# dmlc/xgboost

Hardware: AMD Instinct MI355X
Metric: boosting_rounds_per_sec (higher is better)
Workload: dtype fp32; 1 GPU; model=higgs-1m-hist, rows_per_gpu=1000000, n_features=28, max_depth=8, max_bin=256, objective=binary:logistic, parallelism=dp1, device=cuda

## Files before the change

### xgboost_amd/backend/gpu.py

```python
from __future__ import annotations

from typing import List, Optional, Sequence, Tuple

import numpy as np
import torch

from .. import collective
from ..data import QuantizedMatrix
from ..params import TrainParam
from ..splits import SplitEntry, feature_set_mask
from .cpu import GradQuantizer

LDS_MAX_GROUP_BINS = 8192
TARGET_HIST_TASKS = 2048
MIN_ROWS_PER_TASK = 1024
HIST_MAX_GROUP_FEATURES = 1024


def _check_bin_dtype(gidx: torch.Tensor) -> None:
    if gidx.dtype not in (torch.uint8, torch.int16):
        raise ValueError(
            f"GPU kernels take uint8 or 16-bit bin matrices, got "
            f"{gidx.dtype}: a feature has more than 65535 local bin ids "
            f"(lower max_bin or the category count, or train on the CPU)")
# ... 455 lines not shown
        c8, c16, cld = self._gidx_col_args()
        self.lib.gbt_partition(
            p8, p16, self.qm.n_features, c8, c16, cld, self.hip.ptr(ridx),
            self.hip.ptr(self._ridx_out), self.hip.ptr(tasks), len(tasks_np),
            self.hip.ptr(feat_t), self.hip.ptr(sbin_t), self.hip.ptr(dleft_t),
            self.hip.ptr(cat_bits_t), self.hip.ptr(cat_off_t),
            self.hip.ptr(self.n_bins_feat), self.hip.ptr(cnt_t),
            self.hip.stream())
        self.lib.gbt_copy_ranges(
            self.hip.ptr(self._ridx_out), self.hip.ptr(ridx),
            self.hip.ptr(tasks), len(tasks_np), self.hip.stream())
        final = cnt_t.cpu().numpy()
        out = []
        for i, (s, e) in enumerate(segments):
            mid = int(final[i, 0])
            assert mid == int(final[i, 1]), (
                f"partition counters disagree: {final[i]}")
            out.append(((s, mid), (mid, e)))
        return out

    def grow_tree_native(self, qgpair: torch.Tensor, tree, param,
                         quantizer, monotone: Optional[np.ndarray],
                         root_sums: torch.Tensor,
                         feature_mask: Optional[np.ndarray] = None):
        import ctypes
        if not hasattr(self.lib, "gbt_grow_tree"):
            return None
        if param.max_depth <= 0 or param.max_depth > 14:
            return None
        n_rows = qgpair.shape[0]
        max_build = max(1, 1 << max(param.max_depth - 2, 0))
        pool_rows = 2 * max_build
        pool_bytes = pool_rows * self.n_bins * 16
        if pool_bytes > (32 << 30):
            return None
        dev = self.device
        ws = getattr(self, "_native_ws", None)
        if ws is None or ws["pool_rows"] < pool_rows or ws["n"] < n_rows:
            ws = {
                "pool_rows": pool_rows, "n": n_rows,
                "ridx": torch.empty(n_rows, dtype=torch.int32, device=dev),
                "ridx_out": torch.empty(n_rows, dtype=torch.int32,
                                        device=dev),
                "pool_a": torch.empty((pool_rows, self.n_bins, 2),
                                      dtype=torch.int64, device=dev),
                "pool_b": torch.empty((pool_rows, self.n_bins, 2),
                                      dtype=torch.int64, device=dev),
# ... 63 lines not shown
                       for t in (ws["pool_a"], ws["pool_b"])]
            if ws["wt_ws"] is not None:
                w = ws["wt_ws"]
                regions.append((w.data_ptr(), w.numel(), w))

            def _allreduce(ptr, n_elems):
                addr = ctypes.addressof(ptr.contents)
                for base, nbytes, t in regions:
                    if base <= addr < base + nbytes:
                        off = addr - base
                        i64 = t.view(torch.uint8).view(-1)[
                            off:off + 8 * n_elems].view(torch.int64)
                        collective.allreduce_sum_(i64)
                        return
                raise RuntimeError("allreduce pointer outside workspaces")

            cb = self.hip.ALLREDUCE_FN(_allreduce)
        p8, p16 = self._gidx_ptrs()
        c8, c16, cld = self._gidx_col_args()
        ma = getattr(quantizer, "maxabs_dev", None)
        out_scales = np.zeros(2, dtype=np.float64)
        gsc = quantizer.g_scale if ma is None else 0.0
        hsc = quantizer.h_scale if ma is None else 0.0
        qg_st = ws["qg_stage"][:n_rows]
        qg_st.copy_(qgpair.view(n_rows, 2))
        ws["rs_stage"].copy_(root_sums.view(-1)[:2])
        if ma is not None:
            ws["ma_stage"].copy_(ma.view(-1)[:2])
        rc = self.lib.gbt_grow_tree(
            ws["driver"], p8, p16, self.qm.n_features, c8, c16, n_rows,
            self.hip.ptr(qg_st),
            self.hip.ptr(self.cut_ptrs),
            cut_values_host.ctypes.data_as(ctypes.c_void_p),
            cut_ptrs_host.ctypes.data_as(ctypes.c_void_p),
            self.hip.ptr(self.n_bins_feat),
            self.hip.ptr(self.feat_group_start),
            self.hip.ptr(self.bin_group_start), self.n_groups,
            self.max_group_bins, self.use_shared, self.n_bins,
            self.hip.ptr(ws["ridx"]), self.hip.ptr(ws["ridx_out"]),
            self.hip.ptr(ws["pool_a"]), self.hip.ptr(ws["pool_b"]),
            self.hip.ptr(ws["eval_gain"]), self.hip.ptr(ws["eval_bin"]),
            self.hip.ptr(ws["eval_dir"]), self.hip.ptr(ws["eval_lsum"]),
            self.hip.ptr(ws["eval_best"]), self.hip.ptr(ws["pos"]),
            max_build,
            self.hip.ptr(ws["hist_tasks"]), ws["hist_tasks_cap"],
            self.hip.ptr(ws["wt_ws"]),
            0 if ws["wt_ws"] is None else ws["wt_ws"].numel(),
            ws["wt_max_ptasks"],
            self.hip.ptr(ws["rs_stage"]),
            self.hip.ptr(ws["ma_stage"]) if ma is not None else None,
            out_scales.ctypes.data_as(ctypes.c_void_p),
            gsc, hsc,
            param.reg_lambda, param.reg_alpha, param.max_delta_step,
            param.min_child_weight, param.gamma, param.eta, param.max_depth,
            mono_dev, mono_host, fmask_ptr, cb,
            *[host[k].ctypes.data_as(ctypes.c_void_p) for k in (
                "left", "right", "parent", "split_index", "split_cond",
                "default_left", "loss_chg", "sum_hess", "base_weight")],
            self.hip.stream())
        if rc in (-9998, -9999):
            return None
        if rc <= 0:
            raise RuntimeError(f"gbt_grow_tree failed: rc={rc}")
        if ma is not None:
            quantizer.g_scale = float(out_scales[0])
            quantizer.h_scale = float(out_scales[1])
        n = rc
        tree._ensure(n)
        tree.n_nodes = n
        tree.left[:n] = host["left"][:n]
        tree.right[:n] = host["right"][:n]
        tree.parent[:n] = host["parent"][:n]
        tree.split_index[:n] = host["split_index"][:n]
# ... 722 lines not shown
```

### xgboost_amd/core.py

```python
from __future__ import annotations

import json
import os
from typing import Any, Dict, List, Optional, Sequence, Tuple

import numpy as np
import torch

from . import collective
from .backend.cpu import CpuOps, GradQuantizer
from .data import DMatrix
from .grower import TreeGrower
from .metrics import create_metric
from .objectives import Objective, create_objective
from .params import (TrainParam, canonicalize, check_unknown,
                     make_train_param)
from .tree_model import RegTree

VERSION = (3, 5, 0)


def _resolve_device(params: Dict[str, Any]) -> torch.device:
    dev = str(params.get("device", "cpu"))
    if "device" not in params and params.get("gpu_id") is not None:
# ... 463 lines not shown
        lib.gbt_gpair_fused(
            obj_id, hip_ops.ptr(margin.contiguous().view(-1)),
            hip_ops.ptr(ent["labels"]), hip_ops.ptr(ent["weights"]),
            spw, n, hip_ops.ptr(ent["gh"]), hip_ops.ptr(ent["maxabs"]),
            hip_ops.stream())
        m = ent["maxabs"]
        if collective.is_distributed():
            collective.allreduce_max_(m)
        quantizer = GradQuantizer.__new__(GradQuantizer)
        quantizer.g_scale = None
        quantizer.h_scale = None
        quantizer.maxabs_dev = m
        if "rootsum" not in ent:
            ent["rootsum"] = torch.zeros(2, dtype=torch.int64,
                                         device=margin.device)
        else:
            ent["rootsum"].zero_()
        lib.gbt_quantize(hip_ops.ptr(ent["gh"]), n, 0.0, 0.0,
                         hip_ops.ptr(m), hip_ops.ptr(ent["qg"]),
                         hip_ops.ptr(ent["rootsum"]), hip_ops.stream())
        if collective.is_distributed():
            collective.allreduce_sum_(ent["rootsum"])
        quantizer.root_sums_dev = ent["rootsum"]
        seed = (self.seed + iteration if not self.seed_per_iteration
                else self.seed + iteration * 2654435761)
        tree = RegTree(self.n_features)
        grower = TreeGrower(ops, self.tparam, quantizer, n, seed=seed,
                            monotone=self._monotone_array(),
                            interaction=tp.interaction_constraints,
                            feature_weights=dtrain.info.feature_weights)
        tree, positions = grower.grow(ent["qg"], tree)
        self.trees.append(tree)
        self.tree_info.append(0)
        self.iteration_indptr.append(self.iteration_indptr[-1] + 1)
        leaf_np = tree.split_cond[:tree.n_nodes].copy()
        if hasattr(ops, "stager") and hasattr(lib, "gbt_margin_add") \
                and positions.device == margin.device:
            (leaf_vals,) = ops.stager.upload([leaf_np])
            mc = margin.contiguous()
            lib.gbt_margin_add(hip_ops.ptr(mc), hip_ops.ptr(positions),
                               hip_ops.ptr(leaf_vals), n,
                               mc.stride(0), 0, hip_ops.stream())
            if mc.data_ptr() != margin.data_ptr():
                margin.copy_(mc)
        else:
            leaf_vals = torch.as_tensor(leaf_np, device=margin.device)
# ... 928 lines not shown
```

### xgboost_amd/grower.py

```python
from __future__ import annotations

import dataclasses
import heapq
from typing import Dict, List, Optional, Sequence, Tuple

import numpy as np
import torch

from .backend.cpu import GradQuantizer
from .params import TrainParam
from .splits import SplitEntry, calc_weight, feature_set_mask
from .tree_model import RegTree


class ColumnSampler:

    def __init__(self, n_features: int, param: TrainParam, seed: int,
                 feature_weights: Optional[np.ndarray] = None):
        self.rng = np.random.RandomState(seed & 0x7FFFFFFF)
        self.n_features = n_features
        self.param = param
        self.weights = (np.asarray(feature_weights, dtype=np.float64)
                        if feature_weights is not None else None)
        feats = np.arange(n_features)
# ... 115 lines not shown
        p = self.param
        ops = self.ops
        if not hasattr(ops, "grow_tree_native"):
            return None
        if (self.cat_mask is not None or self.interaction is not None
                or p.colsample_bylevel < 1.0 or p.colsample_bynode < 1.0):
            return None
        fmask = None
        if p.colsample_bytree < 1.0:
            fmask = np.zeros(ops.qm.n_features, np.uint8)
            fmask[self.col_sampler.tree_set] = 1
        needs_replay = p.grow_policy == "lossguide" or p.max_leaves > 0
        if needs_replay:
            if p.max_depth <= 0 or p.max_depth > 14:
                return None
            if p.max_leaves > 0 and (1 << p.max_depth) > 16 * p.max_leaves:
                return None
        rs = getattr(self.quantizer, "root_sums_dev", None)
        if rs is None:
            from . import collective
            rs = qgpair.to(torch.int64).sum(dim=0).contiguous()
            if collective.is_distributed():
                collective.allreduce_sum_(rs)
        out = ops.grow_tree_native(qgpair, tree, p, self.quantizer,
                                   self.monotone, rs, feature_mask=fmask)
        if out is None or not needs_replay:
            return out
        dtree, pos = out
        return self._policy_replay(dtree, pos, p)

    def _policy_replay(self, dt: RegTree, pos: torch.Tensor,
                       param) -> Tuple[RegTree, torch.Tensor]:
        import heapq
        n = dt.n_nodes
        internal = dt.left[:n] >= 0
        gains = getattr(dt, "_gain64", None)
        if gains is None:
            gains = dt.loss_chg[:n].astype(np.float64)
        nt = RegTree(dt.n_features)
        nt._ensure(n)
        new_of = np.full(n, -1, np.int32)
        new_of[0] = 0
        nt.base_weight[0] = dt.base_weight[0]
        nt.sum_hess[0] = dt.sum_hess[0]
        nt.left[0] = nt.right[0] = nt.parent[0] = -1
        state = {"n_new": 1, "n_leaves": 1, "seq": 0}
        heap: List[Tuple[float, int, int, int]] = []

# ... 485 lines not shown
```

### xgboost_amd/ops/__init__.py

```python
from __future__ import annotations

import ctypes
import os
from typing import Optional

import torch

_HERE = os.path.dirname(os.path.abspath(__file__))
_LIB_PATH = os.path.join(_HERE, "libgbt_hip.so")
_lib: Optional[ctypes.CDLL] = None

_c = ctypes
_p = _c.c_void_p
_i = _c.c_int
_i64 = _c.c_int64
_f = _c.c_float
_d = _c.c_double

_SIGS = {
    "gbt_hist": [_p, _p, _i, _p, _p, _p, _i, _p, _i, _p, _p, _i, _i, _p, _i, _p, _p],
    "gbt_partition": [_p, _p, _i, _p, _p, _i64, _p, _p, _p, _i, _p, _p, _p,
                      _p, _p, _p, _p, _p],
    "gbt_evaluate_masked": [_p, _i, _i, _i, _p, _p, _p, _d, _d, _d, _d, _d,
                            _d, _p, _p, _i, _p, _p, _p, _p, _p, _p, _p, _i,
                            _p],
    "gbt_evaluate_ref": [_p, _i, _i, _i, _p, _p, _p, _d, _d, _d, _d, _d,
                         _d, _p, _p, _i, _p, _p, _p, _p, _p, _p, _p, _i,
                         _p],
    "gbt_compress": [_p, _i64, _i, _p, _p, _p, _f, _i, _p, _p, _p],
    "gbt_predict": [_p, _i64, _i, _f, _i, _p, _p, _p, _p, _p, _p, _p, _p,
                    _p, _p, _i, _i, _p, _p, _p],
    "gbt_predict_q": [_p, _i, _i64, _i, _f, _i, _p, _p, _p, _p, _p, _p, _p,
                      _p, _i, _i, _p, _p, _p],
    "gbt_predict_csr": [_p, _p, _p, _i64, _i, _p, _p, _p, _p, _p, _p, _p,
                        _i, _i, _p, _p, _i, _i, _p],
    "gbt_leaf_partition": [_p, _p, _i, _p, _p, _p],
    "gbt_leaf_decide": [_p, _p, _i, _p, _p, _i64, _p, _p, _i, _p, _p, _p,
                        _p, _p, _p, _p],
    "gbt_copy_ranges": [_p, _p, _p, _i, _p],
    "gbt_select_best": [_p, _p, _p, _p, _i, _i, _p, _p, _p],
    "gbt_mt_evaluate": [_p, _i, _i, _i, _i, _p, _p, _p, _p,
                        _d, _d, _d, _d, _p, _p, _p, _p, _p],
    "gbt_gpair_fused": [_i, _p, _p, _p, _f, _i64, _p, _p, _p],
    "gbt_quantize": [_p, _i64, _d, _d, _p, _p, _p, _p],
    "gbt_margin_add": [_p, _p, _p, _i64, _i, _i, _p],
    "gbt_hist_cpu": [_p, _p, _i, _p, _p, _p, _p, _i, _p, _p, _i],
    "gbt_partition_cpu": [_p, _p, _i, _p, _i64, _i64, _i, _i, _i, _p, _i,
                          _i, _p],
    "gbt_evaluate_cpu": [_p, _i, _i, _i, _p, _p, _d, _d, _d, _d, _d, _d,
                         _p, _p, _p, _p],
# ... 97 lines not shown
```

### xgboost_amd/ops/cpp/driver.hip

```cpp
#include "gbt_kernels.h"

#include <hip/hip_runtime.h>

#include <algorithm>
#include <cmath>
#include <cstdio>
#include <cstdlib>
#include <cstring>
#include <vector>

namespace {

#define HIP_CHECK(x)                                    \
  do {                                                  \
    hipError_t err__ = (x);                             \
    if (err__ != hipSuccess) return -(int)err__;        \
  } while (0)

constexpr int kErrReplayDiverged = -9991;
constexpr int kErrRootTasksCap = -9996;
constexpr int kErrArenaTooSmall = -9997;
constexpr int kCapacityTaskGenLds = -9998;
constexpr int kCapacityHistPool = -9999;

// ... 132 lines not shown
    readback_cap = want;
    return 0;
  }
  ~DriverCtx() {
    for (int i = 0; i < PinnedRing::kSlots; ++i) {
      if (ring.host[i]) hipHostFree(ring.host[i]);
      if (ring.dev[i]) hipFree(ring.dev[i]);
    }
    if (readback_host) hipHostFree(readback_host);
    if (wt_graph) (void)hipGraphExecDestroy(wt_graph);
    if (gstream) (void)hipStreamDestroy(gstream);
    if (gevent) (void)hipEventDestroy(gevent);
  }
};

bool WtGraphEnabled() {
  static int v = [] {
    const char* e = getenv("GBT_WT_GRAPH");
    return e ? atoi(e) : 1;
  }();
  return v != 0;
}

constexpr long long kHistMinRows = 2048;
long long HistTasksTarget() {
  static long long v = [] {
    const char* e = getenv("GBT_HIST_TASKS");
    long long t = e ? atoll(e) : 256;
    return t >= 64 && t <= 16384 ? t : 256;
  }();
  return v;
}

long long PartMinRows() {
  static long long v = [] {
    const char* e = getenv("GBT_PART_ROWS");
    long long r = e ? atoll(e) : 4096;
    return r >= 1024 && r <= 65536 && (r & (r - 1)) == 0 ? r : 4096;
  }();
  return v;
}

struct Node {
  int nid;
  int seg_begin, seg_end;
  long long gq, hq;
// ... 173 lines not shown
  }
  __syncthreads();
  const long long rpt = s_rpt;
  const int total_tasks = s_total_tasks;
  for (int t = threadIdx.x; t < max_tasks; t += blockDim.x) {
    if (t >= total_tasks) {
      out_tasks[t] = BlockTask{0, 0, 0, 0};
      continue;
    }
    int lo = 0, hi = k - 1;
    while (lo < hi) {
      const int mid = (lo + hi + 1) >> 1;
      if (s_pref[mid] <= t) lo = mid; else hi = mid - 1;
    }
    const int j = lo;
    const long long idx = t - s_pref[j];
    const int b = s_begin[j] + (int)(idx * rpt);
    const int e = (int)std::min<long long>((long long)b + rpt,
                                           (long long)s_end[j]);
    out_tasks[t] = BlockTask{j, b, e, 0};
  }
}

__global__ void HistTaskGenKernel(const int32_t* __restrict__ counters,
                                  const int32_t* __restrict__ desc, int k,
                                  long long min_rows, long long target_tasks,
                                  int max_tasks,
                                  BlockTask* __restrict__ out_tasks,
                                  int64_t* __restrict__ ps ,
                                  const int32_t* __restrict__ kp_dev,
                                  int32_t* __restrict__ seg_out,
                                  int zero_n,
                                  uint8_t* __restrict__ mode_out
                                  ) {
  if (kp_dev != nullptr) k = *kp_dev;
  if (ps != nullptr) {
    const int zn = max(4 * k, zero_n);
    for (int i = threadIdx.x; i < zn; i += blockDim.x) ps[i] = 0;
  }
  __shared__ int s_begin[kMaxSplitNodes], s_end[kMaxSplitNodes];
  for (int j = threadIdx.x; j < k; j += blockDim.x) {
    const int pb = desc[4 * j], pe = desc[4 * j + 1];
    const int split = counters[2 * desc[4 * j + 2]];
    int mode = desc[4 * j + 3];
    if (mode == 2) mode = (split - pb) <= (pe - split) ? 1 : 0;
    s_begin[j] = mode ? pb : split;
    s_end[j] = mode ? split : pe;
    if (mode_out != nullptr) mode_out[j] = (uint8_t)mode;
    if (seg_out != nullptr) {
      seg_out[2 * j] = s_begin[j];
      seg_out[2 * j + 1] = s_end[j];
      seg_out[2 * (k + j)] = mode ? split : pb;
      seg_out[2 * (k + j) + 1] = mode ? pe : split;
    }
  }
  SplitSegmentsIntoTasks(s_begin, s_end, k, min_rows, target_tasks, max_tasks,
                         out_tasks);
}

__global__ __launch_bounds__(256) void ApplyKernel(
    const int64_t* __restrict__ best,
    const int32_t* __restrict__ segs,
    const int32_t* __restrict__ kn_dev,
    const int32_t* __restrict__ kp_prev_dev,
    const int64_t* __restrict__ ps_prev,
    double gamma_, const int32_t* __restrict__ cut_ptrs,
    long long min_rows, long long target_tasks, int max_ptasks,
    int32_t* __restrict__ kn_out, int32_t* __restrict__ kp_out,
    int32_t* __restrict__ feat, int32_t* __restrict__ sbin,
    uint8_t* __restrict__ dl, int32_t* __restrict__ cnt,
    BlockTask* __restrict__ out_tasks, int32_t* __restrict__ desc,
    int64_t* __restrict__ parent_ps, int32_t* __restrict__ parent_slot,
    int choice_global,
    const float* __restrict__ maxabs,
    const int8_t* __restrict__ monotone,
    double lam, double alpha, double mds,
    const double* __restrict__ bounds_prev,
    double* __restrict__ bounds_out,
    const uint8_t* __restrict__ mode_prev) {
  __shared__ int s_order[kMaxSplitNodes];
// ... 335 lines not shown
  ar.o_cnt = carve((size_t)pool * 8);
  ar.o_ptasks = carve((size_t)wt_max_ptasks * sizeof(BlockTask));
  ar.o_pps = carve((size_t)pool * 16);
  ar.o_pslot = carve((size_t)pool * 4);
  ar.o_ps[0] = carve((size_t)pool * 16);
  ar.o_ps[1] = carve((size_t)pool * 16);
  ar.o_bnd[0] = has_mono ? carve((size_t)pool * 16) : 0;
  ar.o_bnd[1] = has_mono ? carve((size_t)pool * 16) : 0;
  ar.total = off;
  return ar;
}

struct WtChain {
  WtArena ar;
  char* w;
  int n_root_tasks;
  long long root_rpt;
  int wt_max_htasks;
  int n_ptasks;
  template <typename T>
  T* at(size_t off) const { return (T*)(w + off); }
};

int EnqueueChain(const GrowArgs& a, const WtChain& c, hipStream_t cs) {
  const WtArena& ar = c.ar;
  const bool has_mono = a.has_mono();
  const int choice_global = (a.allreduce != nullptr || has_mono) ? 1 : 0;
  const long long hist_row = a.hist_row();
  const int pool = ar.pool;
  int64_t* best_rec = c.at<int64_t>(ar.o_best);
  int32_t* seg_rec = c.at<int32_t>(ar.o_seg);
  int32_t* kn_arr = c.at<int32_t>(ar.o_kn);
  int32_t* kp_arr = c.at<int32_t>(ar.o_kp);
  int32_t* d_desc = c.at<int32_t>(ar.o_desc);
  int32_t* d_feat = c.at<int32_t>(ar.o_feat);
  int32_t* d_sbin = c.at<int32_t>(ar.o_sbin);
  uint8_t* d_dl = c.at<uint8_t>(ar.o_dl);
  int32_t* d_cnt = c.at<int32_t>(ar.o_cnt);
  BlockTask* d_pt = c.at<BlockTask>(ar.o_ptasks);
  int64_t* d_pps = c.at<int64_t>(ar.o_pps);
  int32_t* d_pslot = c.at<int32_t>(ar.o_pslot);
  uint8_t* d_mode = c.at<uint8_t>(ar.o_mode);
  int64_t* ps_bufs[2] = {c.at<int64_t>(ar.o_ps[0]), c.at<int64_t>(ar.o_ps[1])};
  double* bnd_bufs[2] = {has_mono ? c.at<double>(ar.o_bnd[0]) : nullptr,
                         has_mono ? c.at<double>(ar.o_bnd[1]) : nullptr};
  const int8_t* mono = has_mono ? a.monotone_dev : nullptr;
  int32_t* cr = a.ridx;
  int32_t* alt = a.ridx_out;
  int64_t* cp = a.hist_pool_a;
// ... 23 lines not shown
  for (int L = 0; L + 1 < a.max_depth; ++L) {
    const size_t rec_in = L == 0 ? 0 : ar.rec(L - 1);
    const int64_t* bl = best_rec + rec_in * 6;
    const int32_t* sl = seg_rec + rec_in * 2;
    int64_t* bo = best_rec + ar.rec(L) * 6;
    int32_t* so = seg_rec + ar.rec(L) * 2;
    int64_t* ps_next = ps_bufs[L & 1];
    const int cap_kids = (int)std::min<long long>(2LL << L, (long long)pool);
    hipLaunchKernelGGL(ApplyKernel, dim3(1), dim3(256), 0, cs, bl, sl,
                       kn_arr + L, kp_arr + L, ps_prev, a.gamma,
                       a.cut_ptrs_dev, PartMinRows(), (long long)2048,
                       c.n_ptasks, kn_arr + L + 1, kp_arr + L + 1, d_feat,
                       d_sbin, d_dl, d_cnt, d_pt, d_desc, d_pps, d_pslot,
                       choice_global, a.maxabs_dev, mono, a.reg_lambda,
                       a.reg_alpha, a.max_delta_step,
                       (L == 0 || !has_mono) ? nullptr
                                             : bnd_bufs[(L - 1) & 1],
                       bnd_bufs[L & 1],
                       L == 0 ? nullptr : d_mode + (size_t)(L - 1) * pool);
    gbt_partition(a.gidx8, a.gidx16, a.n_features, a.gidx8_col, a.gidx16_col,
                  a.n_rows, cr, alt, d_pt, c.n_ptasks, d_feat, d_sbin,
                  d_dl, nullptr, nullptr, a.n_bins_feat_dev, d_cnt, cs);
    std::swap(cr, alt);
    hipLaunchKernelGGL(HistTaskGenKernel, dim3(1), dim3(256), 0, cs, d_cnt,
                       d_desc, 0, kHistMinRows, HistTasksTarget(),
                       c.wt_max_htasks, a.hist_tasks_dev, ps_next,
                       kp_arr + L + 1, so,
                       a.allreduce != nullptr ? 2 * cap_kids : 0,
                       d_mode + (size_t)L * pool);
    {
      const long long zn = (long long)cap_kids * hist_row;
      int zb = (int)std::min<long long>((zn + 255) / 256, 4096);
      hipLaunchKernelGGL(ZeroI64Kernel, dim3(zb), dim3(256), 0, cs, np2, zn);
    }
    gbt_hist(a.gidx8, a.gidx16, a.n_features, a.qgpair, cr, a.hist_tasks_dev,
             c.wt_max_htasks, np2, a.n_bins, a.feat_group_start_dev,
             a.bin_group_start_dev, a.n_groups, a.max_group_bins,
             a.cut_ptrs_dev, a.use_shared, ps_next, cs);
    if (a.allreduce) {
      a.allreduce((long long*)np2, (long long)(cap_kids / 2) * hist_row);
      a.allreduce((long long*)ps_next, (long long)cap_kids);
    }
    {
      const long long total = (long long)(cap_kids / 2 + 1) * hist_row;
      int blocks = (int)std::min<long long>((total + 255) / 256, 4096);
      hipLaunchKernelGGL(SubtractHistKernel, dim3(blocks), dim3(256), 0, cs,
                         cp, np2, np2, d_pslot, (int)hist_row, 0, ps_next,
                         d_pps, kp_arr + L + 1);
    }
    gbt_evaluate_masked(np2, cap_kids, a.n_bins, a.n_features, a.cut_ptrs_dev,
                        ps_next, a.maxabs_dev, 0.0, 0.0, a.reg_lambda,
                        a.reg_alpha, a.max_delta_step, a.min_child_weight,
                        mono, bnd_bufs[L & 1], 0 , a.fmask_dev,
                        nullptr, a.eval_gain, a.eval_bin, a.eval_dir,
                        a.eval_lsum, kn_arr + L + 1, 0, cs);
    gbt_select_best(a.eval_gain, a.eval_bin, a.eval_dir, a.eval_lsum,
                    cap_kids, a.n_features, bo, kn_arr + L + 1, cs);
    ps_prev = ps_next;
    std::swap(cp, np2);
  }
  return 0;
}

GraphKey ChainKey(const GrowArgs& a, const WtChain& c) {
  typedef unsigned long long U;
  auto db = [](double d) {
    U u;
    memcpy(&u, &d, 8);
    return u;
  };
  return {(U)a.gidx8, (U)a.gidx16, (U)a.gidx8_col, (U)a.gidx16_col,
          (U)a.qgpair, (U)a.cut_ptrs_dev, (U)a.n_bins_feat_dev,
          (U)a.feat_group_start_dev, (U)a.bin_group_start_dev, (U)a.ridx,
          (U)a.ridx_out, (U)a.hist_pool_a, (U)a.hist_pool_b, (U)a.eval_gain,
          (U)a.eval_bin, (U)a.eval_dir, (U)a.eval_lsum, (U)a.hist_tasks_dev,
          (U)a.wt_ws, (U)a.root_sums_dev, (U)a.maxabs_dev, (U)a.monotone_dev,
          (U)a.fmask_dev, (U)a.ctx->readback_host, (U)a.n_rows,
          (U)a.n_features, (U)a.n_bins, (U)a.use_shared, (U)a.n_groups,
          (U)a.max_group_bins, (U)a.max_depth, (U)a.max_nodes_level,
          (U)a.wt_max_ptasks, (U)a.hist_tasks_cap, (U)c.n_root_tasks,
          (U)c.root_rpt, (U)PartMinRows(), (U)c.n_ptasks, (U)c.wt_max_htasks,
          (U)a.has_mono(), db(a.reg_lambda), db(a.reg_alpha),
          db(a.max_delta_step), db(a.min_child_weight), db(a.gamma)};
}

int GrowWholeTree(const GrowArgs& a, TreeOut* out,
                  std::vector<LeafSeg>* leaves) {
  DriverCtx* ctx = a.ctx;
  WtChain c{};
  c.ar = MakeWtArena(a.max_depth, 2 * a.max_nodes_level, a.wt_max_ptasks,
                     a.has_mono());
  const WtArena& ar = c.ar;
  if ((long long)ar.total > a.wt_ws_bytes) return kErrArenaTooSmall;
  c.w = (char*)a.wt_ws;
  c.root_rpt = RootRowsPerTask(a.n_rows, kHistMinRows, HistTasksTarget());
  c.n_root_tasks = RootTaskCount(a.n_rows, c.root_rpt);
  if (c.n_root_tasks > a.hist_tasks_cap) return kErrRootTasksCap;
  c.wt_max_htasks = (int)std::min<long long>(
      std::min<long long>(a.n_rows / kHistMinRows, HistTasksTarget()) +
          a.max_nodes_level + 1,
      (long long)a.hist_tasks_cap);
  c.n_ptasks = (int)std::min<long long>(
      a.n_rows / PartMinRows() + ar.pool + 2, (long long)a.wt_max_ptasks);
  if (int e = ctx->ensure_readback(ar.r_total)) return e;
  char* rb = (char*)ctx->readback_host;

// ... 509 lines not shown
```

### xgboost_amd/ops/cpp/evaluate.hip

```cpp
#include "gbt_kernels.h"
#include "split_gain.h"

#include <algorithm>

namespace {

__device__ __forceinline__ long long ShflUpLL(long long v, int delta) {
  return __shfl_up(v, delta, 64);
}

__device__ __forceinline__ void WaveArgmax(Best* best) {
  for (int off = 32; off > 0; off >>= 1) {
    Best other;
    other.gain = __shfl_down(best->gain, off, 64);
    other.bin = __shfl_down(best->bin, off, 64);
    other.dir = __shfl_down(best->dir, off, 64);
    other.lg = __shfl_down(best->lg, off, 64);
    other.lh = __shfl_down(best->lh, off, 64);
    if (other.bin >= 0 && (best->bin < 0 || Better(other, *best)))
      *best = other;
  }
}

struct EvalArgs {
// ... 30 lines not shown

__device__ __forceinline__ bool NarrowOwns(const EvalArgs& a, int width,
                                           bool is_cat) {
  return a.narrow_max > 0 && width <= a.narrow_max && !is_cat;
}

__device__ __forceinline__ void SetScales(const EvalArgs& a, FeatCtx* c) {
  double g_scale = a.g_scale, h_scale = a.h_scale;
  if (a.maxabs != nullptr) {
    g_scale = a.maxabs[0] > 0.f ? 1073741824.0 / (double)a.maxabs[0] : 1.0;
    h_scale = a.maxabs[1] > 0.f ? 1073741824.0 / (double)a.maxabs[1] : 1.0;
  }
  c->inv_g = 1.0 / g_scale;
  c->inv_h = 1.0 / h_scale;
}

__device__ __forceinline__ void SetParentGain(FeatCtx* c) {
  const double pw = CalcWeight(c->pg * c->inv_g, c->ph * c->inv_h, c->p);
  c->parent_gain =
      GainGivenWeight(c->pg * c->inv_g, c->ph * c->inv_h, pw, c->p);
}

template <bool kNarrow>
__device__ __forceinline__ bool SetupFeature(const EvalArgs& a, int node,
                                             int f, bool writer,
                                             FeatCtx* c) {
  c->out_idx = (size_t)node * a.n_features + f;
  c->fb0 = a.cut_ptrs[f];
  c->fb1 = a.cut_ptrs[f + 1];
  c->is_cat = a.cat_feature && a.cat_feature[f];
  if (NarrowOwns(a, c->fb1 - c->fb0, c->is_cat) != kNarrow) return false;
  if (a.feature_mask != nullptr &&
      a.feature_mask[(size_t)node * a.mask_stride + f] == 0) {
    if (writer) {
      a.out_gain[c->out_idx] = -INFINITY;
      a.out_bin[c->out_idx] = -1;
    }
    return false;
  }
  c->p.lam = a.reg_lambda;
  c->p.alpha = a.reg_alpha;
  c->p.mds = a.max_delta_step;
  c->p.mcw = a.min_child_weight;
  c->p.lo = a.node_bounds ? a.node_bounds[2 * node] : -INFINITY;
  c->p.hi = a.node_bounds ? a.node_bounds[2 * node + 1] : INFINITY;
  c->mono = a.monotone ? (int)a.monotone[f] : 0;
  c->pg = a.parent_sums[2 * node];
  c->ph = a.parent_sums[2 * node + 1];
  c->nh = a.hist + (size_t)node * a.n_bins * 2;
  if (!kNarrow) {
    SetScales(a, c);
    SetParentGain(c);
  }
  return true;
}

__device__ __forceinline__ void WriteBest(const EvalArgs& a, size_t out_idx,
                                          const Best& best) {
  a.out_gain[out_idx] = best.gain;
  a.out_bin[out_idx] = best.bin;
  a.out_dir[out_idx] = (uint8_t)best.dir;
  a.out_lsum[2 * out_idx] = best.lg;
  a.out_lsum[2 * out_idx + 1] = best.lh;
}

__device__ void EvaluateFeatureWave(const EvalArgs& a, const FeatCtx& c,
                                    int lane) {
  const int64_t* nh = c.nh;
  const int fb0 = c.fb0, fb1 = c.fb1;
  const long long pg = c.pg, ph = c.ph;

// ... 51 lines not shown
    }
  }

  WaveArgmax(&best);
  if (lane == 0) WriteBest(a, c.out_idx, best);
}

}

__global__ __launch_bounds__(64) void EvaluateRefKernel(EvalArgs a) {
  const int node = blockIdx.y;
  if (a.k_dev != nullptr && node >= *a.k_dev) return;
  const int lane = threadIdx.x;
  for (int f = blockIdx.x; f < a.n_features; f += gridDim.x) {
    FeatCtx c;
    if (!SetupFeature<false>(a, node, f, lane == 0, &c)) continue;
    EvaluateFeatureWave(a, c, lane);
  }
}

constexpr int kEvalBlock = 256;
constexpr int kEvalWaves = kEvalBlock / 64;

__global__ __launch_bounds__(kEvalBlock) void EvaluateKernel(EvalArgs a) {
  __shared__ long long s_tg[kEvalWaves], s_th[kEvalWaves];
  __shared__ double s_gain[kEvalWaves];
  __shared__ int s_key[kEvalWaves];
  const int node = blockIdx.y;
  if (a.k_dev != nullptr && node >= *a.k_dev) return;
  const int tid = threadIdx.x;
  const int lane = tid & 63;
  const int wave = tid >> 6;
  for (int f = blockIdx.x; f < a.n_features; f += gridDim.x) {
    FeatCtx c;
    if (!SetupFeature<false>(a, node, f, tid == 0, &c)) continue;
    const int width = c.fb1 - c.fb0;
    if (width > kEvalBlock) {
      if (wave == 0) EvaluateFeatureWave(a, c, lane);
      continue;
    }
    const int b = c.fb0 + tid;
    const bool valid = tid < width;
    const long long own_g = valid ? (long long)c.nh[2 * b] : 0;
    const long long own_h = valid ? (long long)c.nh[2 * b + 1] : 0;
    long long sg = own_g, sh = own_h;
    for (int off = 1; off < 64; off <<= 1) {
      const long long tg = ShflUpLL(sg, off);
      const long long th = ShflUpLL(sh, off);
      if (lane >= off) {
        sg += tg;
        sh += th;
      }
    }
    if (lane == 63) {
      s_tg[wave] = sg;
      s_th[wave] = sh;
    }
    __syncthreads();
    long long fg = 0, fh = 0;
    for (int w = 0; w < kEvalWaves; ++w) {
      const long long tg = s_tg[w], th = s_th[w];
      if (w < wave) {
        sg += tg;
        sh += th;
      }
      fg += tg;
      fh += th;
// ... 28 lines not shown
      win_gain = take ? og : win_gain;
      win_key = take ? ok : win_key;
    }
    if (lane == 0) {
      s_gain[wave] = win_gain;
      s_key[wave] = win_key;
    }
    __syncthreads();
    win_gain = s_gain[0];
    win_key = s_key[0];
    for (int w = 1; w < kEvalWaves; ++w) {
      const double og = s_gain[w];
      const int ok = s_key[w];
      const bool take = og > win_gain || (og == win_gain && ok < win_key);
      win_gain = take ? og : win_gain;
      win_key = take ? ok : win_key;
    }
    if (win_key == none) {
      if (tid == 0) WriteBest(a, c.out_idx, best);
    } else if (my_key == win_key) {
      WriteBest(a, c.out_idx, best);
    }
  }
}

__global__ __launch_bounds__(256) void EvaluateNarrowKernel(EvalArgs a) {
  FeatCtx c;
  SetScales(a, &c);
  const int kn = (a.k_dev != nullptr) ? *a.k_dev : a.n_nodes;
  const long long total = (long long)kn * a.n_features;
  const long long stride = (long long)gridDim.x * blockDim.x;
  for (long long idx = (long long)blockIdx.x * blockDim.x + threadIdx.x;
       idx < total; idx += stride) {
    const int node = (int)(idx / a.n_features);
    const int f = (int)(idx % a.n_features);
    if (!SetupFeature<true>(a, node, f, true, &c)) continue;
    long long fg = 0, fh = 0;
    for (int b = c.fb0; b < c.fb1; ++b) {
      fg += c.nh[2 * b];
      fh += c.nh[2 * b + 1];
    }
    Best best{-INFINITY, -1, 0, 0, 0};
    if (fh == 0 && fg == 0) {
      WriteBest(a, c.out_idx, best);
      continue;
    }
// ... 141 lines not shown
                 parent_sums, maxabs, g_scale, h_scale, reg_lambda, reg_alpha,
                 max_delta_step, min_child_weight, monotone, node_bounds,
                 mask_stride, feature_mask, cat_feature, out_gain, out_bin,
                 out_dir, out_lsum, k_dev, narrow_max, stream);
}

extern "C" void gbt_evaluate_ref(
    const int64_t* hist, int n_nodes, int n_bins, int n_features,
    const int32_t* cut_ptrs, const int64_t* parent_sums,
    const float* maxabs, double g_scale,
    double h_scale, double reg_lambda, double reg_alpha,
    double max_delta_step, double min_child_weight, const int8_t* monotone,
    const double* node_bounds, int mask_stride,
    const uint8_t* feature_mask,
    const uint8_t* cat_feature, double* out_gain, int32_t* out_bin,
    uint8_t* out_dir, int64_t* out_lsum, const int32_t* k_dev,
    int narrow_max, hipStream_t stream) {
  LaunchEvaluate(true, hist, n_nodes, n_bins, n_features, cut_ptrs,
                 parent_sums, maxabs, g_scale, h_scale, reg_lambda, reg_alpha,
                 max_delta_step, min_child_weight, monotone, node_bounds,
                 mask_stride, feature_mask, cat_feature, out_gain, out_bin,
                 out_dir, out_lsum, k_dev, narrow_max, stream);
}
```

### xgboost_amd/ops/cpp/gbt_kernels.h

```cpp
#pragma once
#include <hip/hip_runtime.h>
#include <cstdint>

struct BlockTask {
  int32_t out_slot;
  int32_t row_begin;
  int32_t row_end;
  int32_t pad;
};

extern "C" {

void gbt_hist(const uint8_t* gidx8, const uint16_t* gidx16,
              int n_features, const int32_t* qgpair ,
              const int32_t* ridx, const BlockTask* tasks, int n_tasks,
              int64_t* out_hist , int n_bins,
              const int32_t* feat_group_start,
              const int32_t* bin_group_start,
              int n_groups, int max_group_bins,
              const int32_t* cut_ptrs,
              int use_shared,
              int64_t* node_sums,
              hipStream_t stream);

// ... 25 lines not shown
    const uint8_t* feature_mask,
    const uint8_t* cat_feature,
    double* out_gain,
    int32_t* out_bin,
    uint8_t* out_dir,
    int64_t* out_lsum,
    const int32_t* k_dev,
    int narrow_max,
    hipStream_t stream);

void gbt_evaluate_ref(const int64_t* hist, int n_nodes, int n_bins,
                      int n_features, const int32_t* cut_ptrs,
                      const int64_t* parent_sums, const float* maxabs,
                      double g_scale, double h_scale, double reg_lambda,
                      double reg_alpha, double max_delta_step,
                      double min_child_weight, const int8_t* monotone,
                      const double* node_bounds, int mask_stride,
                      const uint8_t* feature_mask,
                      const uint8_t* cat_feature, double* out_gain,
                      int32_t* out_bin, uint8_t* out_dir,
                      int64_t* out_lsum, const int32_t* k_dev,
                      int narrow_max, hipStream_t stream);

void gbt_compress(const float* X, int64_t n_rows, int n_features,
                  const float* cut_values, const int32_t* cut_ptrs,
                  const uint8_t* cat_feature, float missing_value,
                  int missing_is_nan,
                  uint8_t* out8, uint16_t* out16, hipStream_t stream);

void gbt_predict(const float* X, int64_t n_rows, int n_features,
                 float missing_value, int missing_is_nan,
                 const int32_t* tree_offsets,
                 const int32_t* left, const int32_t* right,
                 const int32_t* split_index, const float* split_cond,
                 const uint8_t* default_left, const uint8_t* split_type,
                 const int32_t* cat_offsets,
                 const uint32_t* cat_bits,
                 const int32_t* tree_group,
                 int n_trees, int n_groups,
                 float* out_margin,
                 int32_t* out_leaf,
                 hipStream_t stream);

void gbt_predict_q(const void* X, int kind, int64_t n_rows, int n_features,
                   float missing_value, int missing_is_nan,
                   const int32_t* n_bins,
// ... 50 lines not shown
```

Measured before the change: 1130 rounds/s.

## Fuse histogram subtraction into split evaluation and task-gen with zeroing

Adds a fused evaluate kernel that computes sibling histograms by parent-minus-built subtraction inside the evaluation blocks, writing them out while scanning, and a prep kernel that combines hist task generation with zeroing the next-level histogram pool (only half the slots). It also skips staging copies of gradient pairs and root sums when inputs are stable device tensors. This is meant to remove several kernel launches and a separate pass over histogram memory per level, at the cost of more complex kernels and extra per-feature syncs for wide features.

Measured after the change: 1181 rounds/s (median of 6 runs). +4.6%, better.

```diff
diff --git a/xgboost_amd/backend/gpu.py b/xgboost_amd/backend/gpu.py
--- a/xgboost_amd/backend/gpu.py
+++ b/xgboost_amd/backend/gpu.py
@@ -501,7 +501,8 @@
     def grow_tree_native(self, qgpair: torch.Tensor, tree, param,
                          quantizer, monotone: Optional[np.ndarray],
                          root_sums: torch.Tensor,
-                         feature_mask: Optional[np.ndarray] = None):
+                         feature_mask: Optional[np.ndarray] = None,
+                         stable_inputs: bool = False):
         import ctypes
         if not hasattr(self.lib, "gbt_grow_tree"):
             return None
@@ -611,11 +612,22 @@
         out_scales = np.zeros(2, dtype=np.float64)
         gsc = quantizer.g_scale if ma is None else 0.0
         hsc = quantizer.h_scale if ma is None else 0.0
-        qg_st = ws["qg_stage"][:n_rows]
-        qg_st.copy_(qgpair.view(n_rows, 2))
-        ws["rs_stage"].copy_(root_sums.view(-1)[:2])
-        if ma is not None:
-            ws["ma_stage"].copy_(ma.view(-1)[:2])
+        if (stable_inputs and qgpair.is_contiguous()
+                and qgpair.dtype == torch.int32
+                and root_sums.is_contiguous()
+                and root_sums.dtype == torch.int64
+                and (ma is None or (ma.is_contiguous()
+                                    and ma.dtype == torch.float32))):
+            qg_st, rs_st, ma_st = qgpair, root_sums, ma
+        else:
+            qg_st = ws["qg_stage"][:n_rows]
+            qg_st.copy_(qgpair.view(n_rows, 2))
+            rs_st = ws["rs_stage"]
+            rs_st.copy_(root_sums.view(-1)[:2])
+            ma_st = None
+            if ma is not None:
+                ma_st = ws["ma_stage"]
+                ma_st.copy_(ma.view(-1)[:2])
         rc = self.lib.gbt_grow_tree(
             ws["driver"], p8, p16, self.qm.n_features, c8, c16, n_rows,
             self.hip.ptr(qg_st),
@@ -636,8 +648,8 @@
             self.hip.ptr(ws["wt_ws"]),
             0 if ws["wt_ws"] is None else ws["wt_ws"].numel(),
             ws["wt_max_ptasks"],
-            self.hip.ptr(ws["rs_stage"]),
-            self.hip.ptr(ws["ma_stage"]) if ma is not None else None,
+            self.hip.ptr(rs_st),
+            self.hip.ptr(ma_st) if ma is not None else None,
             out_scales.ctypes.data_as(ctypes.c_void_p),
             gsc, hsc,
             param.reg_lambda, param.reg_alpha, param.max_delta_step,
diff --git a/xgboost_amd/core.py b/xgboost_amd/core.py
--- a/xgboost_amd/core.py
+++ b/xgboost_amd/core.py
@@ -509,6 +509,7 @@
         if collective.is_distributed():
             collective.allreduce_sum_(ent["rootsum"])
         quantizer.root_sums_dev = ent["rootsum"]
+        quantizer.stable_inputs = True
         seed = (self.seed + iteration if not self.seed_per_iteration
                 else self.seed + iteration * 2654435761)
         tree = RegTree(self.n_features)
diff --git a/xgboost_amd/grower.py b/xgboost_amd/grower.py
--- a/xgboost_amd/grower.py
+++ b/xgboost_amd/grower.py
@@ -161,8 +161,10 @@
             rs = qgpair.to(torch.int64).sum(dim=0).contiguous()
             if collective.is_distributed():
                 collective.allreduce_sum_(rs)
+        stable = bool(getattr(self.quantizer, "stable_inputs", False))
         out = ops.grow_tree_native(qgpair, tree, p, self.quantizer,
-                                   self.monotone, rs, feature_mask=fmask)
+                                   self.monotone, rs, feature_mask=fmask,
+                                   stable_inputs=stable)
         if out is None or not needs_replay:
             return out
         dtree, pos = out
diff --git a/xgboost_amd/ops/__init__.py b/xgboost_amd/ops/__init__.py
--- a/xgboost_amd/ops/__init__.py
+++ b/xgboost_amd/ops/__init__.py
@@ -26,6 +26,9 @@
                             _p],
     "gbt_evaluate_ref": [_p, _i, _i, _i, _p, _p, _p, _d, _d, _d, _d, _d,
                          _d, _p, _p, _i, _p, _p, _p, _p, _p, _p, _p, _i,
+                         _p],
+    "gbt_evaluate_sub": [_p, _i, _i, _i, _p, _p, _p, _d, _d, _d, _d, _d,
+                         _d, _p, _p, _p, _p, _p, _p, _p, _p, _p, _p, _p,
                          _p],
     "gbt_compress": [_p, _i64, _i, _p, _p, _p, _f, _i, _p, _p, _p],
     "gbt_predict": [_p, _i64, _i, _f, _i, _p, _p, _p, _p, _p, _p, _p, _p,
diff --git a/xgboost_amd/ops/cpp/driver.hip b/xgboost_amd/ops/cpp/driver.hip
--- a/xgboost_amd/ops/cpp/driver.hip
+++ b/xgboost_amd/ops/cpp/driver.hip
@@ -178,6 +178,16 @@
   return v != 0;
 }
 
+constexpr int kFusePrep = 1;
+constexpr int kFuseSub = 2;
+int WtFuseMask() {
+  static int v = [] {
+    const char* e = getenv("GBT_WT_FUSE");
+    return (e ? atoi(e) : ~0) & (kFusePrep | kFuseSub);
+  }();
+  return v;
+}
+
 constexpr long long kHistMinRows = 2048;
 long long HistTasksTarget() {
   static long long v = [] {
@@ -397,8 +407,8 @@
   }
 }
 
-__global__ void HistTaskGenKernel(const int32_t* __restrict__ counters,
-                                  const int32_t* __restrict__ desc, int k,
+__device__ inline void HistTaskGen(const int32_t* __restrict__ counters,
+                                   const int32_t* __restrict__ desc, int k,
                                   long long min_rows, long long target_tasks,
                                   int max_tasks,
                                   BlockTask* __restrict__ out_tasks,
@@ -431,6 +441,35 @@
   }
   SplitSegmentsIntoTasks(s_begin, s_end, k, min_rows, target_tasks, max_tasks,
                          out_tasks);
+}
+
+__global__ void HistTaskGenKernel(const int32_t* counters, const int32_t* desc,
+                                  int k, long long min_rows,
+                                  long long target_tasks, int max_tasks,
+                                  BlockTask* out_tasks, int64_t* ps,
+                                  const int32_t* kp_dev, int32_t* seg_out,
+                                  int zero_n, uint8_t* mode_out) {
+  HistTaskGen(counters, desc, k, min_rows, target_tasks, max_tasks, out_tasks,
+              ps, kp_dev, seg_out, zero_n, mode_out);
+}
+
+__global__ __launch_bounds__(256) void HistPrepKernel(
+    const int32_t* counters, const int32_t* desc, long long min_rows,
+    long long target_tasks, int max_tasks, BlockTask* out_tasks, int64_t* ps,
+    const int32_t* kp_dev, int32_t* seg_out, uint8_t* mode_out,
+    int64_t* __restrict__ hist, long long hist_row ,
+    int max_slots) {
+  if (blockIdx.x == 0) {
+    HistTaskGen(counters, desc, 0, min_rows, target_tasks, max_tasks,
+                out_tasks, ps, kp_dev, seg_out, 0, mode_out);
+    return;
+  }
+  const long long n2 = (long long)min(*kp_dev, max_slots) * (hist_row / 2);
+  const long long stride = (long long)(gridDim.x - 1) * blockDim.x;
+  longlong2* h2 = (longlong2*)hist;
+  for (long long i = (long long)(blockIdx.x - 1) * blockDim.x + threadIdx.x;
+       i < n2; i += stride)
+    h2[i] = make_longlong2(0, 0);
 }
 
 __global__ __launch_bounds__(256) void ApplyKernel(
@@ -812,9 +851,16 @@
   T* at(size_t off) const { return (T*)(w + off); }
 };
 
+int ChainFuseMask(const GrowArgs& a) {
+  return a.allreduce != nullptr ? 0 : WtFuseMask();
+}
+
 int EnqueueChain(const GrowArgs& a, const WtChain& c, hipStream_t cs) {
   const WtArena& ar = c.ar;
   const bool has_mono = a.has_mono();
+  const int fuse = ChainFuseMask(a);
+  const bool fuse_prep = (fuse & kFusePrep) != 0;
+  const bool fuse_sub = (fuse & kFuseSub) != 0;
   const int choice_global = (a.allreduce != nullptr || has_mono) ? 1 : 0;
   const long long hist_row = a.hist_row();
   const int pool = ar.pool;
@@ -884,13 +930,22 @@
                   a.n_rows, cr, alt, d_pt, c.n_ptasks, d_feat, d_sbin,
                   d_dl, nullptr, nullptr, a.n_bins_feat_dev, d_cnt, cs);
     std::swap(cr, alt);
-    hipLaunchKernelGGL(HistTaskGenKernel, dim3(1), dim3(256), 0, cs, d_cnt,
-                       d_desc, 0, kHistMinRows, HistTasksTarget(),
-                       c.wt_max_htasks, a.hist_tasks_dev, ps_next,
-                       kp_arr + L + 1, so,
-                       a.allreduce != nullptr ? 2 * cap_kids : 0,
-                       d_mode + (size_t)L * pool);
-    {
+    if (fuse_prep) {
+      const long long zn2 = (long long)(cap_kids / 2) * (hist_row / 2);
+      const int zb = (int)std::min<long long>((zn2 + 511) / 512, 2048);
+      hipLaunchKernelGGL(HistPrepKernel, dim3(1 + std::max(zb, 1)), dim3(256),
+                         0, cs, d_cnt, d_desc, kHistMinRows,
+                         HistTasksTarget(), c.wt_max_htasks, a.hist_tasks_dev,
+                         ps_next, kp_arr + L + 1, so,
+                         d_mode + (size_t)L * pool, np2, hist_row,
+                         cap_kids / 2);
+    } else {
+      hipLaunchKernelGGL(HistTaskGenKernel, dim3(1), dim3(256), 0, cs, d_cnt,
+                         d_desc, 0, kHistMinRows, HistTasksTarget(),
+                         c.wt_max_htasks, a.hist_tasks_dev, ps_next,
+                         kp_arr + L + 1, so,
+                         a.allreduce != nullptr ? 2 * cap_kids : 0,
+                         d_mode + (size_t)L * pool);
       const long long zn = (long long)cap_kids * hist_row;
       int zb = (int)std::min<long long>((zn + 255) / 256, 4096);
       hipLaunchKernelGGL(ZeroI64Kernel, dim3(zb), dim3(256), 0, cs, np2, zn);
@@ -903,19 +958,27 @@
       a.allreduce((long long*)np2, (long long)(cap_kids / 2) * hist_row);
       a.allreduce((long long*)ps_next, (long long)cap_kids);
     }
-    {
+    if (fuse_sub) {
+      gbt_evaluate_sub(np2, cap_kids, a.n_bins, a.n_features, a.cut_ptrs_dev,
+                       ps_next, a.maxabs_dev, 0.0, 0.0, a.reg_lambda,
+                       a.reg_alpha, a.max_delta_step, a.min_child_weight, mono,
+                       bnd_bufs[L & 1], a.fmask_dev, cp, d_pslot, d_pps,
+                       a.eval_gain, a.eval_bin, a.eval_dir, a.eval_lsum,
+                       kp_arr + L + 1, cs);
+    } else {
       const long long total = (long long)(cap_kids / 2 + 1) * hist_row;
       int blocks = (int)std::min<long long>((total + 255) / 256, 4096);
       hipLaunchKernelGGL(SubtractHistKernel, dim3(blocks), dim3(256), 0, cs,
                          cp, np2, np2, d_pslot, (int)hist_row, 0, ps_next,
                          d_pps, kp_arr + L + 1);
-    }
-    gbt_evaluate_masked(np2, cap_kids, a.n_bins, a.n_features, a.cut_ptrs_dev,
-                        ps_next, a.maxabs_dev, 0.0, 0.0, a.reg_lambda,
-                        a.reg_alpha, a.max_delta_step, a.min_child_weight,
-                        mono, bnd_bufs[L & 1], 0 , a.fmask_dev,
-                        nullptr, a.eval_gain, a.eval_bin, a.eval_dir,
-                        a.eval_lsum, kn_arr + L + 1, 0, cs);
+      gbt_evaluate_masked(np2, cap_kids, a.n_bins, a.n_features,
+                          a.cut_ptrs_dev, ps_next, a.maxabs_dev, 0.0, 0.0,
+                          a.reg_lambda, a.reg_alpha, a.max_delta_step,
+                          a.min_child_weight, mono, bnd_bufs[L & 1],
+                          0 , a.fmask_dev, nullptr, a.eval_gain,
+                          a.eval_bin, a.eval_dir, a.eval_lsum, kn_arr + L + 1,
+                          0, cs);
+    }
     gbt_select_best(a.eval_gain, a.eval_bin, a.eval_dir, a.eval_lsum,
                     cap_kids, a.n_features, bo, kn_arr + L + 1, cs);
     ps_prev = ps_next;
@@ -942,8 +1005,9 @@
           (U)a.max_group_bins, (U)a.max_depth, (U)a.max_nodes_level,
           (U)a.wt_max_ptasks, (U)a.hist_tasks_cap, (U)c.n_root_tasks,
           (U)c.root_rpt, (U)PartMinRows(), (U)c.n_ptasks, (U)c.wt_max_htasks,
-          (U)a.has_mono(), db(a.reg_lambda), db(a.reg_alpha),
-          db(a.max_delta_step), db(a.min_child_weight), db(a.gamma)};
+          (U)a.has_mono(), (U)ChainFuseMask(a), db(a.reg_lambda),
+          db(a.reg_alpha), db(a.max_delta_step), db(a.min_child_weight),
+          db(a.gamma)};
 }
 
 int GrowWholeTree(const GrowArgs& a, TreeOut* out,
diff --git a/xgboost_amd/ops/cpp/evaluate.hip b/xgboost_amd/ops/cpp/evaluate.hip
--- a/xgboost_amd/ops/cpp/evaluate.hip
+++ b/xgboost_amd/ops/cpp/evaluate.hip
@@ -76,9 +76,9 @@
 }
 
 template <bool kNarrow>
-__device__ __forceinline__ bool SetupFeature(const EvalArgs& a, int node,
-                                             int f, bool writer,
-                                             FeatCtx* c) {
+__device__ __forceinline__ bool SetupFeature(
+    const EvalArgs& a, int node, int f, bool writer, FeatCtx* c,
+    bool own_sums = false, long long sum_g = 0, long long sum_h = 0) {
   c->out_idx = (size_t)node * a.n_features + f;
   c->fb0 = a.cut_ptrs[f];
   c->fb1 = a.cut_ptrs[f + 1];
@@ -99,8 +99,8 @@
   c->p.lo = a.node_bounds ? a.node_bounds[2 * node] : -INFINITY;
   c->p.hi = a.node_bounds ? a.node_bounds[2 * node + 1] : INFINITY;
   c->mono = a.monotone ? (int)a.monotone[f] : 0;
-  c->pg = a.parent_sums[2 * node];
-  c->ph = a.parent_sums[2 * node + 1];
+  c->pg = own_sums ? sum_g : a.parent_sums[2 * node];
+  c->ph = own_sums ? sum_h : a.parent_sums[2 * node + 1];
   c->nh = a.hist + (size_t)node * a.n_bins * 2;
   if (!kNarrow) {
     SetScales(a, c);
@@ -198,27 +198,79 @@
 constexpr int kEvalBlock = 256;
 constexpr int kEvalWaves = kEvalBlock / 64;
 
-__global__ __launch_bounds__(kEvalBlock) void EvaluateKernel(EvalArgs a) {
+struct SubArgs {
+  const int64_t* parents;
+  const int32_t* parent_slot;
+  const int64_t* parent_ps;
+  int64_t* hist;
+  int64_t* ps;
+};
+
+template <bool kSub>
+__device__ __forceinline__ void EvaluateBlock(const EvalArgs& a,
+                                              const SubArgs& s) {
   __shared__ long long s_tg[kEvalWaves], s_th[kEvalWaves];
   __shared__ double s_gain[kEvalWaves];
   __shared__ int s_key[kEvalWaves];
   const int node = blockIdx.y;
-  if (a.k_dev != nullptr && node >= *a.k_dev) return;
+  int k = 0;
+  if (kSub) {
+    k = *a.k_dev;
+    if (node >= 2 * k) return;
+  } else if (a.k_dev != nullptr && node >= *a.k_dev) {
+    return;
+  }
   const int tid = threadIdx.x;
   const int lane = tid & 63;
   const int wave = tid >> 6;
+  const bool sub = kSub && node >= k;
+  const size_t hist_row = (size_t)a.n_bins * 2;
+  long long sub_g = 0, sub_h = 0;
+  const int64_t* par_h = nullptr;
+  const int64_t* built_h = nullptr;
+  int64_t* dst_h = nullptr;
+  if (sub) {
+    const int j = node - k;
+    sub_g = s.parent_ps[2 * j] - a.parent_sums[2 * j];
+    sub_h = s.parent_ps[2 * j + 1] - a.parent_sums[2 * j + 1];
+    if (blockIdx.x == 0 && tid == 0) {
+      s.ps[2 * node] = sub_g;
+      s.ps[2 * node + 1] = sub_h;
+    }
+    par_h = s.parents + (size_t)s.parent_slot[j] * hist_row;
+    built_h = a.hist + (size_t)j * hist_row;
+    dst_h = s.hist + (size_t)node * hist_row;
+  }
   for (int f = blockIdx.x; f < a.n_features; f += gridDim.x) {
     FeatCtx c;
-    if (!SetupFeature<false>(a, node, f, tid == 0, &c)) continue;
+    if (!SetupFeature<false>(a, node, f, tid == 0, &c, sub, sub_g, sub_h))
+      continue;
     const int width = c.fb1 - c.fb0;
     if (width > kEvalBlock) {
+      if (sub) {
+        for (int b = c.fb0 + tid; b < c.fb1; b += kEvalBlock) {
+          dst_h[2 * b] = par_h[2 * b] - built_h[2 * b];
+          dst_h[2 * b + 1] = par_h[2 * b + 1] - built_h[2 * b + 1];
+        }
+        __syncthreads();
+      }
       if (wave == 0) EvaluateFeatureWave(a, c, lane);
       continue;
     }
     const int b = c.fb0 + tid;
     const bool valid = tid < width;
-    const long long own_g = valid ? (long long)c.nh[2 * b] : 0;
-    const long long own_h = valid ? (long long)c.nh[2 * b + 1] : 0;
+    long long own_g = 0, own_h = 0;
+    if (sub) {
+      if (valid) {
+        own_g = par_h[2 * b] - built_h[2 * b];
+        own_h = par_h[2 * b + 1] - built_h[2 * b + 1];
+        dst_h[2 * b] = own_g;
+        dst_h[2 * b + 1] = own_h;
+      }
+    } else if (valid) {
+      own_g = c.nh[2 * b];
+      own_h = c.nh[2 * b + 1];
+    }
     long long sg = own_g, sh = own_h;
     for (int off = 1; off < 64; off <<= 1) {
       const long long tg = ShflUpLL(sg, off);
@@ -293,6 +345,15 @@
       WriteBest(a, c.out_idx, best);
     }
   }
+}
+
+__global__ __launch_bounds__(kEvalBlock) void EvaluateKernel(EvalArgs a) {
+  EvaluateBlock<false>(a, SubArgs{});
+}
+
+__global__ __launch_bounds__(kEvalBlock) void EvaluateSubKernel(EvalArgs a,
+                                                                SubArgs s) {
+  EvaluateBlock<true>(a, s);
 }
 
 __global__ __launch_bounds__(256) void EvaluateNarrowKernel(EvalArgs a) {
@@ -480,3 +541,25 @@
                  mask_stride, feature_mask, cat_feature, out_gain, out_bin,
                  out_dir, out_lsum, k_dev, narrow_max, stream);
 }
+
+extern "C" void gbt_evaluate_sub(
+    int64_t* hist, int n_nodes, int n_bins, int n_features,
+    const int32_t* cut_ptrs, int64_t* ps, const float* maxabs,
+    double g_scale, double h_scale, double reg_lambda, double reg_alpha,
+    double max_delta_step, double min_child_weight, const int8_t* monotone,
+    const double* node_bounds, const uint8_t* feature_mask,
+    const int64_t* parents, const int32_t* parent_slot,
+    const int64_t* parent_ps, double* out_gain, int32_t* out_bin,
+    uint8_t* out_dir, int64_t* out_lsum, const int32_t* k_dev,
+    hipStream_t stream) {
+  const EvalArgs ea{hist, n_nodes, n_bins, n_features, cut_ptrs, ps, maxabs,
+                    k_dev, 0 , g_scale, h_scale, reg_lambda,
+                    reg_alpha, max_delta_step, min_child_weight, monotone,
+                    node_bounds, 0 , feature_mask,
+                    nullptr , out_gain, out_bin, out_dir,
+                    out_lsum};
+  const SubArgs sa{parents, parent_slot, parent_ps, hist, ps};
+  dim3 grid(n_features > 65535 ? 65535 : n_features, n_nodes);
+  hipLaunchKernelGGL(EvaluateSubKernel, grid, dim3(kEvalBlock), 0, stream, ea,
+                     sa);
+}
diff --git a/xgboost_amd/ops/cpp/gbt_kernels.h b/xgboost_amd/ops/cpp/gbt_kernels.h
--- a/xgboost_amd/ops/cpp/gbt_kernels.h
+++ b/xgboost_amd/ops/cpp/gbt_kernels.h
@@ -71,6 +71,18 @@
                       int64_t* out_lsum, const int32_t* k_dev,
                       int narrow_max, hipStream_t stream);
 
+void gbt_evaluate_sub(
+    int64_t* hist , int n_nodes ,
+    int n_bins, int n_features, const int32_t* cut_ptrs,
+    int64_t* ps , const float* maxabs, double g_scale,
+    double h_scale, double reg_lambda, double reg_alpha,
+    double max_delta_step, double min_child_weight, const int8_t* monotone,
+    const double* node_bounds, const uint8_t* feature_mask ,
+    const int64_t* parents, const int32_t* parent_slot ,
+    const int64_t* parent_ps , double* out_gain,
+    int32_t* out_bin, uint8_t* out_dir, int64_t* out_lsum,
+    const int32_t* k_dev , hipStream_t stream);
+
 void gbt_compress(const float* X, int64_t n_rows, int n_features,
                   const float* cut_values, const int32_t* cut_ptrs,
                   const uint8_t* cat_feature, float missing_value,
```
